# sarphiv/nerf-experiments

Measured on AMD Instinct MI355X. Metric: ray-samples/sec (coarse+fine), training step, higher is better.
Workload: dtype fp32

## Files before the change

include/nerf_amd.h:

```cpp
#ifndef NERF_AMD_H
#define NERF_AMD_H

#include <stdint.h>
#include <stddef.h>

#ifdef __cplusplus
extern "C" {
#endif

#define NERF_OK 0
#define NERF_ERR_INVALID_ARG (-1)
#define NERF_ERR_UNSUPPORTED (-2)
#define NERF_ERR_LAUNCH (-3)
#define NERF_ERR_WORKSPACE (-4)

int nerf_abi_version(void);
const char* nerf_status_string(int status);
int64_t nerf_struct_size(int32_t which);
#define NERF_BUILD_DIAG_FUSED 1
#define NERF_BUILD_DIAG_WGRAD 2
int32_t nerf_build_flags(void);

int nerf_composite_fwd(const float* density, int64_t density_stride,
                       const float* color, int64_t color_stride,
// ... 97 lines not shown
                       float* out, int64_t ldo, int32_t epilogue,
                       const float* aux, int64_t ld_aux, void* stream);
int nerf_linear_wgrad_x3(const float* dY, int64_t ld_dy, int32_t N,
                         const nerf_seg* segs, int32_t n_segs, int64_t M,
                         void* workspace, size_t workspace_bytes, int32_t passes, void* stream);
int nerf_linear_wgrad_x3_rows(const float* dY, int64_t ld_dy, const nerf_seg* segs, int64_t M0,
                              const float* dY1, int64_t ld_dy1, const nerf_seg* segs1, int64_t M1,
                              int32_t n_segs, int32_t N, void* workspace, size_t workspace_bytes,
                              int32_t passes, void* stream);
int nerf_linear_wgrad_x3_rays(const float* dY, int64_t ld_dy, const nerf_seg* segs, int64_t M0,
                              const float* dY1, int64_t ld_dy1, const nerf_seg* segs1, int64_t M1,
                              int32_t n_segs, int32_t N, void* workspace, size_t workspace_bytes,
                              float* raysum, int32_t samples_per_ray0, int32_t samples_per_ray1,
                              int32_t passes, void* stream);
int nerf_linear_wgrad_x3_rows_q(const float* dY, int64_t ld_dy, const nerf_seg* segs, int64_t M0,
                                const float* dY1, int64_t ld_dy1, const nerf_seg* segs1, int64_t M1,
                                int32_t n_segs, int32_t N, void* workspace, size_t workspace_bytes,
                                int32_t passes, uint32_t x_split_mask, void* stream);
int nerf_linear_wgrad_x3_rays_q(const float* dY, int64_t ld_dy, const nerf_seg* segs, int64_t M0,
                                const float* dY1, int64_t ld_dy1, const nerf_seg* segs1, int64_t M1,
                                int32_t n_segs, int32_t N, void* workspace, size_t workspace_bytes,
                                float* raysum, int32_t samples_per_ray0, int32_t samples_per_ray1,
                                int32_t passes, uint32_t x_split_mask, void* stream);
int nerf_pack_weight_x3(const float* W, int32_t N, int32_t K_orig, const int32_t* col_map,
                        int32_t Kp, void* Wp_x, void* Wt_x, int32_t ldwt, void* stream);

#define NERF_FUSED_MAX_LAYERS 16
typedef struct nerf_fused_layer {
    int32_t type;
    int32_t N;
    int32_t nb;
    int32_t relu;
    int32_t nseg;
    int32_t seg_kb[2];
    int32_t seg_k[2];
    int32_t seg_rd[2];
    int32_t seg_rows[2];
    int32_t chunk_units;
    int32_t col_idx;
    int64_t seg_ld[2];
    const float* seg_ptr[2];
    float* out;
    int64_t ldo;
    uint8_t* mask;
    float* col_out;
    int64_t img_off;
// ... 245 lines not shown
```

nerf-experiments_amd/csrc/linear_x3.hip:

```cpp
#include "common.h"
#include "param_act.h"

using namespace nerf;

typedef float f32x16 __attribute__((ext_vector_type(16)));
typedef float f4 __attribute__((ext_vector_type(4)));
typedef __bf16 bf16x8 __attribute__((ext_vector_type(8)));
typedef __bf16 bf16x4 __attribute__((ext_vector_type(4)));
typedef unsigned short u16x8 __attribute__((ext_vector_type(8)));

namespace {

constexpr int BK = 32;
constexpr int LDB = BK;

__device__ __forceinline__ int swz(int row, int slot) {
    return (row >> 1) * 64 + ((((row & 1) << 2) | slot) ^ ((row >> 2) & 7)) * 8;
}
constexpr int MAX_SEGS = 4;

struct SegList {
    const float* ptr[MAX_SEGS];
    int64_t ld[MAX_SEGS];
    int k[MAX_SEGS];
// ... 1444 lines not shown
            const int k = wc * 32 * JN + j * 32 + (lane & 31);
#pragma unroll
            for (int r = 0; r < 16; ++r) {
                const int n = wr * 128 + i * 32 + (r & 3) + 8 * (r >> 2) + 4 * (lane >> 5);
                if (n < npad && k < kpad) slab[(size_t)n * kpad + k] = acc[i][j][r];
            }
        }
    float* red = reinterpret_cast<float*>(smem);
    *reinterpret_cast<f4*>(red + (op * 4 + (wave & 3)) * 256 + 4 * lane) = op == 0 ? dbp : dacc;
    if (ROW257 && op == 1 && lane == 0) red[2048 + (wave & 3)] = dbx;
    __syncthreads();
    if (t < 256) {
        const float s = ((red[t] + red[256 + t]) + red[512 + t]) + red[768 + t];
        if (t < npad) a.db_slab[(size_t)split * npad + t] = s;
    } else if (ROW257) {
        const int c = t - 256;
        const float* x = red + 1024;
        slab[(size_t)256 * kpad + c] = ((x[c] + x[256 + c]) + x[512 + c]) + x[768 + c];
        if (c == 0)
            a.db_slab[(size_t)split * npad + 256] = ((red[2048] + red[2049]) + red[2050]) + red[2051];
    }
#undef WT_SRC_ROW
#undef WT_YD_ROW
}

constexpr int SN_T = 512;
constexpr int SN_U = 8;
template <int N4>
__global__ __launch_bounds__(SN_T) void linear_wgrad_smalln_kernel(TNArgs a, int kpad) {
    extern __shared__ __attribute__((aligned(16))) float sn_part[];
    const int split = blockIdx.x;
    const int mbeg = split * a.m_per_split;
    const int mend = min(mbeg + a.m_per_split, a.M);
    const int ktot = a.X.ktot;
    const int qw = ktot >> 2;
    const int rg = SN_T / qw;
    const int t = threadIdx.x;
    const int g = t / qw, q = t - g * qw;
    const bool live = g < rg;
    int xs = 0, xoff = 0;
#pragma unroll
    for (int i = 0; i < MAX_SEGS; ++i)
        if (i < a.X.n && 4 * q >= a.X.koff[i] && 4 * q < a.X.koff[i] + a.X.kp[i]) { xs = i; xoff = 4 * q - a.X.koff[i]; }
    const bool col_ok = live && xoff < pick4(a.X.k, xs);
    const float* xp0 = pick4(a.X.ptr, xs) + xoff;
    const int64_t xld0 = pick4(a.X.ld, xs);
// ... 496 lines not shown
                                           int32_t n_segs, int32_t N, void* workspace, size_t workspace_bytes,
                                           float* raysum, int32_t samples_per_ray0, int32_t samples_per_ray1,
                                           int32_t passes, uint32_t x_split_mask, void* stream) {
    NERF_REQUIRE(raysum != nullptr);
    return wgrad_x3_rows_impl(dY, ld_dy, segs, M0, dY1, ld_dy1, segs1, M1, n_segs, N, workspace, workspace_bytes,
                              raysum, samples_per_ray0, samples_per_ray1, passes, x_split_mask, stream);
}

extern "C" int nerf_linear_wgrad_x3_rays(const float* dY, int64_t ld_dy, const nerf_seg* segs, int64_t M0,
                                         const float* dY1, int64_t ld_dy1, const nerf_seg* segs1, int64_t M1,
                                         int32_t n_segs, int32_t N, void* workspace, size_t workspace_bytes,
                                         float* raysum, int32_t samples_per_ray0, int32_t samples_per_ray1,
                                         int32_t passes, void* stream) {
    return nerf_linear_wgrad_x3_rays_q(dY, ld_dy, segs, M0, dY1, ld_dy1, segs1, M1, n_segs, N, workspace,
                                       workspace_bytes, raysum, samples_per_ray0, samples_per_ray1, passes, 0u, stream);
}

extern "C" int nerf_linear_wgrad_x3(const float* dY, int64_t ld_dy, int32_t N, const nerf_seg* segs, int32_t n_segs,
                                    int64_t M, void* workspace, size_t workspace_bytes, int32_t passes, void* stream) {
    return nerf_linear_wgrad_x3_rows(dY, ld_dy, segs, M, nullptr, 0, nullptr, 0, n_segs, N, workspace,
                                     workspace_bytes, passes, stream);
}

extern "C" int nerf_pack_weight_x3(const float* W, int32_t N, int32_t K_orig, const int32_t* col_map, int32_t Kp,
                                   void* Wp_x, void* Wt_x, int32_t ldwt, void* stream) {
    NERF_REQUIRE(W && col_map && N >= 1 && K_orig >= 1 && Kp >= 1 && (Kp % BK) == 0);
    const int npad = ((N + 127) / 128) * 128;
    if (Wt_x) NERF_REQUIRE(ldwt >= ((N + 31) / 32) * 32 && (ldwt % BK) == 0);
    const int kpad_rows = ((Kp + 127) / 128) * 128 + 128;
    int64_t total = (int64_t)npad * Kp;
    if (Wt_x) {
        const int64_t pad_total = (int64_t)(kpad_rows - Kp) * ldwt;
        if (pad_total > total) total = pad_total;
    }
    hipLaunchKernelGGL(pack_weight_x3_kernel, dim3((unsigned)((total + 255) / 256)), dim3(256), 0, as_stream(stream), W,
                       N, K_orig, col_map, Kp, npad, reinterpret_cast<__bf16*>(Wp_x), reinterpret_cast<__bf16*>(Wt_x),
                       ldwt, kpad_rows);
    NERF_CHECK_LAUNCH();
    return NERF_OK;
}

extern "C" __attribute__((visibility("hidden"))) int32_t nerf_tu_build_flags_linear_x3(void) {
    return NERF_TU_BUILD_FLAGS;
}
```

nerf-experiments_amd/nerf_amd/_lib.py:

```python
from __future__ import annotations

import ctypes
import os

import torch

_HERE = os.path.dirname(os.path.abspath(__file__))
LIB_PATH = os.environ.get("NERF_AMD_LIB", os.path.join(_HERE, "libnerf_amd.so"))

c_f = ctypes.c_float
c_i32 = ctypes.c_int32
c_i64 = ctypes.c_int64
c_u32 = ctypes.c_uint32
c_u64 = ctypes.c_uint64
c_vp = ctypes.c_void_p
c_sz = ctypes.c_size_t

NERF_EPI_BIAS = 1
NERF_EPI_RELU = 2
NERF_EPI_MASK = 4
NERF_EPI_ACCUM = 8
NERF_EPI_MASKBITS = 16
NERF_EPI_MASKOUT = 32
NERF_EPI_NO_PERSIST = 256
# ... 191 lines not shown
                                c_i32, c_vp, c_i64, c_vp]),
    "nerf_linear_wgrad_workspace": (c_sz, [c_i64, c_i32, c_i32]),
    "nerf_linear_wgrad": (c_i32, [c_vp, c_i64, c_i32, ctypes.POINTER(NerfSeg), c_i32, c_i64, c_vp, c_sz, c_vp]),
    "nerf_linear_wgrad_reduce": (c_i32, [c_i64, c_i32, c_i32, c_i32, c_vp, c_vp, c_vp, c_i64, c_vp, c_i32, c_vp]),
    "nerf_pack_weight": (c_i32, [c_vp, c_i32, c_i32, c_vp, c_i32, c_vp, c_vp, c_i32, c_vp]),
    "nerf_linear_fwd_x3": (c_i32, [ctypes.POINTER(NerfSeg), c_i32, c_i64, c_vp, c_i32, c_i32, c_vp, c_vp,
                                   c_i64, c_i32, c_vp, c_i64, c_vp]),
    "nerf_linear_gauss_workspace": (c_sz, [c_i64, c_i32]),
    "nerf_linear_gauss_x3": (c_i32, [ctypes.POINTER(NerfSeg), c_i32, c_i64, c_vp, c_i32, c_i32, c_vp, c_vp, c_i64,
                                     c_i32, c_vp, c_vp, c_i64, c_vp, c_i64, c_vp, c_i32, c_vp, c_sz, c_vp]),
    "nerf_linear_wgrad_x3": (c_i32, [c_vp, c_i64, c_i32, ctypes.POINTER(NerfSeg), c_i32, c_i64, c_vp, c_sz, c_i32,
                                     c_vp]),
    "nerf_linear_wgrad_x3_rows": (c_i32, [c_vp, c_i64, ctypes.POINTER(NerfSeg), c_i64, c_vp, c_i64,
                                          ctypes.POINTER(NerfSeg), c_i64, c_i32, c_i32, c_vp, c_sz, c_i32, c_vp]),
    "nerf_linear_wgrad_x3_rays": (c_i32, [c_vp, c_i64, ctypes.POINTER(NerfSeg), c_i64, c_vp, c_i64,
                                          ctypes.POINTER(NerfSeg), c_i64, c_i32, c_i32, c_vp, c_sz, c_vp, c_i32,
                                          c_i32, c_i32, c_vp]),
    "nerf_linear_wgrad_x3_rows_q": (c_i32, [c_vp, c_i64, ctypes.POINTER(NerfSeg), c_i64, c_vp, c_i64,
                                            ctypes.POINTER(NerfSeg), c_i64, c_i32, c_i32, c_vp, c_sz, c_i32, c_u32,
                                            c_vp]),
    "nerf_linear_wgrad_x3_rays_q": (c_i32, [c_vp, c_i64, ctypes.POINTER(NerfSeg), c_i64, c_vp, c_i64,
                                            ctypes.POINTER(NerfSeg), c_i64, c_i32, c_i32, c_vp, c_sz, c_vp, c_i32,
                                            c_i32, c_i32, c_u32, c_vp]),
    "nerf_pack_weight_x3": (c_i32, [c_vp, c_i32, c_i32, c_vp, c_i32, c_vp, c_vp, c_i32, c_vp]),
    "nerf_mlp_fused_fwd": (c_i32, [ctypes.POINTER(NerfFusedLayer), c_i32, c_vp, c_i64,
                                   ctypes.POINTER(NerfFusedEncoding), c_vp]),
    "nerf_mlp_fused_render": (c_i32, [ctypes.POINTER(NerfFusedLayer), c_i32, c_vp, c_i64,
                                      ctypes.POINTER(NerfFusedEncoding), ctypes.POINTER(NerfFusedComposite), c_vp]),
    "nerf_mlp_fused_run": (c_i32, [ctypes.POINTER(NerfFusedLayer), c_i32, c_vp, c_i64, ctypes.POINTER(NerfFusedEncoding),
                                   ctypes.POINTER(NerfFusedComposite), c_i32, c_vp]),
    "nerf_struct_size": (c_i64, [c_i32]),
    "nerf_build_flags": (c_i32, []),
    "nerf_fused_pack": (c_i32, [ctypes.POINTER(c_vp), c_i32, c_vp, c_vp, c_i64, c_vp, c_vp]),
    "nerf_hashgrid_fwd": (c_i32, [ctypes.POINTER(NerfHashgridParams), c_vp, c_vp, c_vp, c_vp, c_vp, c_i64, c_i32,
                                  c_vp, c_vp, c_i64, c_vp]),
    "nerf_kabsch": (c_i32, [c_vp, c_vp, c_i32, c_i32, c_vp, c_vp, c_vp, c_vp, c_vp]),
    "nerf_pose_rays_fwd": (c_i32, [c_vp, c_vp, c_i32, c_vp, c_vp, c_vp, c_i64, c_f, c_vp, c_vp, c_vp, c_vp, c_vp]),
    "nerf_pose_rays_bwd": (c_i32, [c_vp, c_i32, c_vp, c_vp, c_i64, c_f, c_vp, c_vp, c_vp, c_vp, c_vp, c_vp, c_vp,
                                   c_vp, c_vp]),
    "nerf_prop_cdf": (c_i32, [c_vp, c_i64, c_i64, c_i32, c_vp, c_i64, c_vp]),
    "nerf_prop_sample": (c_i32, [c_vp, c_i64, c_vp, c_i64, c_i64, c_i32, c_i32, c_i32, c_u64, c_u64, c_i32, c_f,
                                 c_f, c_vp, c_vp, c_i64, c_vp]),
    "nerf_prop_loss": (c_i32, [c_vp, c_vp, c_i64, c_vp, c_vp, c_i64, c_i64, c_i32, c_i32, c_f, c_vp, c_f, c_vp,
                               c_i64, c_vp]),
    "nerf_hashgrid_workspace": (c_sz, [ctypes.POINTER(NerfHashgridParams)]),
    "nerf_hashgrid_workspace_n": (c_sz, [ctypes.POINTER(NerfHashgridParams), c_i64]),
# ... 71 lines not shown
```

nerf-experiments_amd/nerf_amd/kernels.py:

```python
from __future__ import annotations

import ctypes
import os
from typing import Sequence

import torch

from . import _lib
from ._lib import NerfPEParams, NerfSeg


class KernelTimer:

    def __init__(self):
        self.records = []

    def bracket(self, tag: str, flops: float = 0.0, nbytes: float = 0.0, fn: str | None = None, launches: int = 1):
        start = torch.cuda.Event(enable_timing=True)
        end = torch.cuda.Event(enable_timing=True)
        start.record()
        self.records.append((tag, flops, nbytes, start, end, fn or tag, launches))
        return end

    def summary(self, by: str = "tag"):
# ... 563 lines not shown
        raise ValueError("linear_wgrad_x3_rows: the blocks' segments differ in width")
    a0, a1 = make_segs(segs), make_segs(segs1)
    kt = sum(k for _, k, _ in segs)
    kpad = sum(pad32(k) for _, k, _ in segs)
    wide = wgrad_single_tile(N4, kpad)
    end = TIMER.bracket("linear_wgrad_x3", 2.0 * (M + M1) * N4 * kt,
                        4.0 * (M + M1) * N4 + _segs_bytes(segs, M) + _segs_bytes(segs1, M1) + 4.0 * N4 * kt,
                        fn=WGRAD_TILE_FN if wide else
                        ("linear_wgrad_smalln_kernel" if N4 <= 16 else "linear_wgrad_x3_kernel")) \
        if TIMER is not None else None
    if x_split_mask:
        st = _lib.load().nerf_linear_wgrad_x3_rows_q(_ptr(dY), dY.stride(0), a0, M, _ptr(dY1), dY1.stride(0), a1, M1,
                                                     len(segs), N4, _ptr(workspace),
                                                     workspace.numel() * workspace.element_size(), passes,
                                                     x_split_mask, _stream(dY.device))
    else:
        st = _lib.load().nerf_linear_wgrad_x3_rows(_ptr(dY), dY.stride(0), a0, M, _ptr(dY1), dY1.stride(0), a1, M1,
                                                   len(segs), N4, _ptr(workspace),
                                                   workspace.numel() * workspace.element_size(), passes,
                                                   _stream(dY.device))
    if end is not None:
        end.record()
    _lib.check(st, "nerf_linear_wgrad_x3_rows")


def linear_wgrad_x3_rays(blocks, N4: int, workspace: torch.Tensor, raysum: torch.Tensor, S0: int, S1: int,
                        passes: int = 3, x_split_mask: int = 0) -> None:
    (dY, segs, M), (dY1, segs1, M1) = blocks
    a0, a1 = make_segs(segs), make_segs(segs1)
    kt = sum(k for _, k, _ in segs)
    if raysum.shape[1] != N4 or not raysum.is_contiguous():
        raise ValueError("linear_wgrad_x3_rays: raysum must be contiguous [rays, N4]")
    end = TIMER.bracket("linear_wgrad_x3", 2.0 * (M + M1) * N4 * kt,
                        4.0 * (M + M1) * N4 + _segs_bytes(segs, M) + _segs_bytes(segs1, M1) + 4.0 * N4 * kt
                        + 4.0 * raysum.numel(), fn=WGRAD_TILE_FN) \
        if TIMER is not None else None
    if x_split_mask:
        st = _lib.load().nerf_linear_wgrad_x3_rays_q(_ptr(dY), dY.stride(0), a0, M, _ptr(dY1), dY1.stride(0), a1, M1,
                                                     len(segs), N4, _ptr(workspace),
                                                     workspace.numel() * workspace.element_size(), _ptr(raysum), S0,
                                                     S1, passes, x_split_mask, _stream(dY.device))
    else:
        st = _lib.load().nerf_linear_wgrad_x3_rays(_ptr(dY), dY.stride(0), a0, M, _ptr(dY1), dY1.stride(0), a1, M1,
                                                   len(segs), N4, _ptr(workspace),
                                                   workspace.numel() * workspace.element_size(), _ptr(raysum), S0,
                                                   S1, passes, _stream(dY.device))
# ... 751 lines not shown
```

nerf-experiments_amd/nerf_amd/mlp.py:

```python
from __future__ import annotations

import math
import os
from dataclasses import dataclass, field

import torch
import torch.nn as nn

from . import kernels as K
from . import mlp_fused
from ._lib import (NERF_EPI_ACCUM, NERF_EPI_BIAS, NERF_EPI_MASK, NERF_EPI_MASKBITS, NERF_EPI_MASKOUT,
                   NERF_EPI_RELU, NERF_EPI_TANH, NERF_EPI_TANH_BWD)


def matmul_precision() -> str:
    if PRECISION_OVERRIDE is not None:
        return PRECISION_OVERRIDE
    p = torch.get_float32_matmul_precision()
    return "fp32" if p == "highest" else ("x1" if p == "medium" else "x3")


def is_split(prec: str) -> bool:
    return prec in ("x3", "x1")

# ... 110 lines not shown
        return None
    rows = [(0, nrow)] if nrow <= 257 else [(n0, min(256, nrow - n0)) for n0 in range(0, nrow, 256)]
    groups, cur, used = [], [], 0
    for j, (_, k, rd) in enumerate(segs):
        if kp[j] > 256 and rd != 1:
            return None
        for c0 in range(0, k, 256):
            c1 = min(c0 + 256, k)
            w = K.pad32(c1 - c0)
            if used + w > 256:
                groups.append(cur)
                cur, used = [], 0
            cur.append((j, c0, c1))
            used += w
    groups.append(cur)
    gk = [sum(K.pad32(c1 - c0) for _, c0, c1 in g) for g in groups]
    if len(rows) > 1 and min(gk) <= 128:
        return None
    if any(not (nb > 128 or k > 128) for _, nb in rows for k in gk):
        return None
    return rows, groups


def _wgrad_tiles(blocks, nrow: int, N4: int, lp, workspace, gW, gb, acc, split, npass: int, q=()) -> None:
    rows, groups = split
    Mt = sum(M for _, _, M in blocks)
    poff = [0]
    for _, k, _ in blocks[0][1]:
        poff.append(poff[-1] + K.pad32(k))

    def piece(segs, j, c0, c1):
        t, k, rd = segs[j]
        return (t, k, rd) if (c0, c1) == (0, k) else (t[:, c0:c1], c1 - c0, rd)

    whole = len(rows) == 1
    for n0, nb in rows:
        nr = nrow if whole else nb
        n4 = N4 if whole else nb
        nvalid = lp.N if whole else min(nb, lp.N - n0)
        for gi, g in enumerate(groups):
            pb = [(dZ if whole else dZ[:, n0:n0 + nb], [piece(segs, j, c0, c1) for j, c0, c1 in g], M)
                  for dZ, segs, M in blocks]
            p0 = poff[g[0][0]] + g[0][1]
            kp = sum(K.pad32(c1 - c0) for _, c0, c1 in g)
            ws = _wgrad_workspace(workspace, Mt, n4, kp)
            qm = _qmask(q, [j for j, _, _ in g])
            if len(pb) > 1:
                K.linear_wgrad_x3_rows(pb, nr, ws, passes=npass, x_split_mask=qm)
            else:
                K.linear_wgrad_x3(pb[0][0], nr, pb[0][1], pb[0][2], ws, passes=npass, x_split_mask=qm)
            K.linear_wgrad_reduce(Mt, n4, kp, nvalid, ws, lp.col_map[p0:p0 + kp], gW[n0:n0 + nvalid],
                                  gb[n0:n0 + nvalid] if gi == 0 else None, accumulate=acc)


def _qmask(q, js) -> int:
    return sum(1 << i for i, j in enumerate(js) if j < len(q) and q[j])


def _wgrad_x3(blocks, nrow: int, N4: int, lp, workspace, gW, gb, acc, npass: int, q=()) -> None:
    segs = blocks[0][1]
    rsplit = _ray_split(blocks, N4) if nrow == N4 else None
    tsplit = _tile_split(segs, nrow) if rsplit is None else None
    if rsplit is not None:
        _wgrad_rays(blocks, N4, lp, workspace, gW, gb, acc, rsplit, npass, q)
    elif tsplit is not None:
        _wgrad_tiles(blocks, nrow, N4, lp, workspace, gW, gb, acc, tsplit, npass, q)
    else:
        Mt = sum(M for _, _, M in blocks)
        qm = _qmask(q, range(len(segs)))
        ws = _wgrad_workspace(workspace, Mt, N4, lp.Kp)
        if len(blocks) > 1:
            K.linear_wgrad_x3_rows(blocks, nrow, ws, passes=npass, x_split_mask=qm)
        else:
            K.linear_wgrad_x3(blocks[0][0], nrow, segs, blocks[0][2], ws, passes=npass, x_split_mask=qm)
        K.linear_wgrad_reduce(Mt, N4, lp.Kp, lp.N, ws, lp.col_map, gW, gb, accumulate=acc)


def wgrad_launches(segs, nrow: int, N4: int, M: int, rays: bool = True):
    rsplit = _ray_split([(None, segs, M)], N4) if rays and nrow == N4 else None
    if rsplit is not None:
        n = len(segs) - 1
        return [(N4, [(j, K.pad32(segs[j][1])) for j in range(n)]), (N4, [(n, K.pad32(segs[n][1]))])]
    tsplit = _tile_split(segs, nrow)
    if tsplit is not None:
        rows, groups = tsplit
        return [(nrow if len(rows) == 1 else nb, [(j, K.pad32(c1 - c0)) for j, c0, c1 in g])
                for _, nb in rows for g in groups]
    return [(nrow, [(j, K.pad32(k)) for j, (_, k, _) in enumerate(segs)])]


SAVE_SPLIT = False


def split_layers(plan, M: int, dir_rd: int) -> frozenset:
    if not SAVE_SPLIT or CAPTURE is not None or not mlp_fused.dgrad_eligible(plan, M):
        return frozenset()
    cols = {li for li, _ in plan.column_outputs}
    out = set()
    for l, lp in enumerate(plan.layers[:-1]):
        if lp.N > 256 or l in plan.outputs or l in cols or lp.keeps_pre or lp.tanh:
            continue
        readers = [(c, si) for c, cl in enumerate(plan.layers) for si, s in enumerate(cl.sources)
                   if s.kind == "act" and s.layer == l]
        if not readers or any(cl.residual == l for cl in plan.layers):
            continue
        ok = True
        for c, si in readers:
            cl = plan.layers[c]
            if c != l + 1 or si != 0 or cl.N == 257:
                ok = False
                break
# ... 416 lines not shown
                    if comp_chain and l == sl and plan.layers[l].out_ld == 260:
                        continue
                    dY[l][:, 256:].zero_()
            if comp_chain:
                comp_rt = (comp, g_rgb, dY[L - 1], dY[sl][:, 256:] if sl >= 0 else None, sl)
            x_out = {}
            for (l, _, _, _, x, *_rest) in fd.steps:
                if x is not None:
                    x_out[l] = torch.empty(M, x.k_pad, device=dev, dtype=torch.float32)
            fd.run(M, g_head, dY, ctx.masks, g_cols, x_out, comp=comp_rt, passes=passes(ctx.prec))
            for (l, _, _, _, x, *_rest) in fd.steps:
                if x is None:
                    continue
                if x.kind == "pos":
                    dpos = x_out[l] if dpos is None else dpos.add_(x_out[l])
                else:
                    ddir = x_out[l] if ddir is None else ddir.add_(x_out[l])

        ws_bytes = 0
        for lp in plan.layers:
            ws_bytes = max(ws_bytes, K.linear_wgrad_workspace_bytes(M, (lp.N + 3) // 4 * 4, lp.Kp))
        workspace = torch.empty((ws_bytes + 3) // 4, device=dev, dtype=torch.float32)

        for li in range(L - 1, -1, -1):
            lp = plan.layers[li]
            if col_grads[li]:
                if dY[li] is None:
                    dY[li] = torch.zeros(M, lp.out_ld, device=dev, dtype=torch.float32)
                elif not owned[li]:
                    dY[li] = dY[li].clone()
                for c, g in col_grads[li]:
                    dY[li][:, c] += g
            dZ = dY[li]
            w = lp.module.weight
            sink = ctx.sink
            if dZ is None:
                if sink is not None:
                    for t in (w, lp.module.bias):
                        g, acc = sink.target(t)
                        if not acc:
                            g.zero_()
                        sink.landed(t)
                    layer_grads[li] = [None, None]
                else:
                    layer_grads[li] = [torch.zeros_like(w), torch.zeros_like(lp.module.bias)]
                layer_grads[li] += [torch.zeros_like(p) for p in lp.pact]
                continue
# ... 16 lines not shown
                segs.append((t, s.k_seg, rd))
            N4 = (lp.N + 3) // 4 * 4
            nrow = lp.N if (lp.N == 257 and WGRAD_ROW257) else N4
            q = tuple(s.kind == "act" and s.layer in ctx.split for s in lp.sources)
            merge = sink is not None and is_split(ctx.prec) and MERGE_PASSES and not gs
            prev = sink.stash.pop((id(plan), li), (None, None))[0] if merge else None
            if merge and prev is None and sink.remaining(w) >= 2:
                sink.stash[(id(plan), li)] = ((dZ, segs, M, nrow, N4, lp, passes(ctx.prec), q), _flush_wgrad)
                layer_grads[li] = [None, None]
            else:
                if sink is not None:
                    gW, acc = sink.target(w)
                    gb, acc_b = sink.target(lp.module.bias)
                    if acc != acc_b:
                        raise RuntimeError("direct gradient sink: weight and bias of one layer out of step")
                else:
                    gW, gb, acc = torch.empty_like(w), torch.empty_like(lp.module.bias), False
                npass = passes(ctx.prec)
                if prev is not None and prev[7] != q:
                    _wgrad_x3([(prev[0], prev[1], prev[2])], nrow, N4, lp, workspace, gW, gb, acc, npass, prev[7])
                    _wgrad_x3([(dZ, segs, M)], nrow, N4, lp, workspace, gW, gb, True, npass, q)
                elif is_split(ctx.prec):
                    wblocks = [(prev[0], prev[1], prev[2]), (dZ, segs, M)] if prev is not None else [(dZ, segs, M)]
                    _wgrad_x3(wblocks, nrow, N4, lp, workspace, gW, gb, acc, npass, q)
                else:
                    K.linear_wgrad(dZ, N4, segs, M, workspace)
                    K.linear_wgrad_reduce(M, N4, lp.Kp, lp.N, workspace, lp.col_map, gW, gb, accumulate=acc)
                if sink is not None:
                    for _ in range(2 if prev is not None else 1):
                        sink.landed(w)
                        sink.landed(lp.module.bias)
                    gW = gb = None
                layer_grads[li] = [gW, gb] + (gs if gs is not None else [])
            if chain:
                continue
            lp.pack(ctx.prec, forward=False)
            a_seg = [(dZ, lp.out_ld, 1)]
            for s, koff in zip(lp.sources, lp.koffs):
                if s.kind == "act":
                    j = s.layer
                    prod = plan.layers[j]
                    if (GAUSS_EPILOGUE and prod.keeps_pre and plan.contributors[j] == 1 and dY[j] is None
                            and not prod.relu and is_split(ctx.prec) and prod.bwd_epilogue_fits(s.k_valid)):
                        dz = torch.empty(M, prod.out_ld, device=dev, dtype=torch.float32)
                        gsj = [torch.empty_like(p) for p in prod.pact]
                        if prod.linear_act_x3(a_seg, M, lp.Wtx, lp.ldwt, s.k_valid, dz, z=pre[j], grads=gsj,
                                              w_row_offset=koff):
                            dY[j] = dz
                            gauss_done[j] = gsj
                            continue
                    epi = 0
                    aux = None
                    if prod.tanh:
                        epi |= NERF_EPI_TANH_BWD
# ... 10 lines not shown
                            aux = acts[j]
                    fresh = dY[j] is None
                    if fresh:
                        dY[j] = torch.empty(M, prod.out_ld, device=dev, dtype=torch.float32)
                    else:
                        epi |= NERF_EPI_ACCUM
                    lp.gemm(ctx.prec, a_seg, M, True, s.k_valid, None, dY[j], epi, aux=aux, row_offset=koff)
                    if fresh and prod.out_ld > s.k_valid:
                        dY[j][:, s.k_valid:].zero_()
                elif s.kind == "pos" and need_pos:
                    if dpos is None:
                        dpos = torch.empty(M, s.k_pad, device=dev, dtype=torch.float32)
                        epi = 0
                    else:
                        epi = NERF_EPI_ACCUM
                    lp.gemm(ctx.prec, a_seg, M, True, s.k_pad, None, dpos, epi, row_offset=koff)
                elif s.kind == "dir" and need_dir:
                    if ddir is None:
                        ddir = torch.empty(M, s.k_pad, device=dev, dtype=torch.float32)
                        epi = 0
                    else:
                        epi = NERF_EPI_ACCUM
                    lp.gemm(ctx.prec, a_seg, M, True, s.k_pad, None, ddir, epi, row_offset=koff)
        if ddir is not None and ctx.dir_rd > 1:
            ddir = ddir.view(-1, ctx.dir_rd, ddir.shape[1]).sum(dim=1)
        if dpos is not None and dpos.shape[1] != ctx.n_pos_cols:
            dpos = dpos[:, :ctx.n_pos_cols]
        if ddir is not None and ddir.shape[1] != ctx.n_dir_cols:
            ddir = ddir[:, :ctx.n_dir_cols]
        param_grads = [g for lg in layer_grads for g in lg]
        return (None, None, dpos, ddir, None, *param_grads)


def nerf_model_plan(n_segments: int, model_segments: nn.ModuleList, model_color: nn.Sequential,
                    hidden_dim: int, pos_dim: int, dir_dim: int, delayed_direction: bool,
                    delayed_density: bool) -> tuple[MLPPlan, int, int]:
    layers: list[LayerPlan] = []
    pos_src = Source("pos", pos_dim, K.pad32(pos_dim))
    dir_src = Source("dir", dir_dim, K.pad32(dir_dim))
    prev = -1
    for i in range(n_segments):
        seg = model_segments[i]
        linears = [m for m in seg.modules() if isinstance(m, nn.Linear)] if isinstance(seg, nn.Sequential) \
            else [seg]
        for j, lin in enumerate(linears):
            srcs: list[Source] = []
# ... 24 lines not shown
```

Measured before the change: 72.15 million.

## Pair two weight-gradient GEMMs sharing the same position input into one kernel

Adds a paired wgrad kernel that reads the shared X (position encoding) tile once and computes weight gradients for two layers (late skip-connection piece and early layer) in a single launch, each using half the waves. The Python backward defers (holds) the late layer's pos-segment wgrad until the matching early layer is reached, then launches the pair. This is meant to remove one pass over X and one launch, and to improve occupancy for the small-K GEMMs. In exchange it allocates an extra workspace per call, makes the bookkeeping more complex, and changes when gradients are marked landed.

After: 72.76 million (median of 6 runs). No clear change (+0.8%).

```diff
diff --git a/include/nerf_amd.h b/include/nerf_amd.h
--- a/include/nerf_amd.h
+++ b/include/nerf_amd.h
@@ -143,6 +143,12 @@
                                 int32_t n_segs, int32_t N, void* workspace, size_t workspace_bytes,
                                 float* raysum, int32_t samples_per_ray0, int32_t samples_per_ray1,
                                 int32_t passes, uint32_t x_split_mask, void* stream);
+int nerf_linear_wgrad_x3_pair(const float* dYa, int64_t ld_dya, const float* dYa1, int64_t ld_dya1,
+                              int32_t Na, int32_t bias_a, void* workspace_a, size_t workspace_a_bytes,
+                              const float* dYb, int64_t ld_dyb, const float* dYb1, int64_t ld_dyb1,
+                              int32_t Nb, int32_t bias_b, void* workspace_b, size_t workspace_b_bytes,
+                              const nerf_seg* segs, int64_t M0, const nerf_seg* segs1, int64_t M1,
+                              int32_t n_segs, int32_t passes, uint32_t x_split_mask, void* stream);
 int nerf_pack_weight_x3(const float* W, int32_t N, int32_t K_orig, const int32_t* col_map,
                         int32_t Kp, void* Wp_x, void* Wt_x, int32_t ldwt, void* stream);
 
diff --git a/nerf-experiments_amd/csrc/linear_x3.hip b/nerf-experiments_amd/csrc/linear_x3.hip
--- a/nerf-experiments_amd/csrc/linear_x3.hip
+++ b/nerf-experiments_amd/csrc/linear_x3.hip
@@ -1490,6 +1490,244 @@
     }
 #undef WT_SRC_ROW
 #undef WT_YD_ROW
+}
+
+constexpr int PT_IMG = 6 * WT_T * 512;
+constexpr int PT_RELAY = 2 * 4 * 4 * 64 * 16;
+struct TNPairArgs {
+    const float* dY[2][2]; int64_t lddy[2][2]; int N[2];
+    const float* X[2]; int64_t ldx[2]; int k, kp;
+    int M, M0, m_per_split;
+    float* slab[2]; float* db_slab[2];
+    int npad[2], kpad;
+};
+
+template <bool X1>
+__global__ __launch_bounds__(512, 1) __attribute__((amdgpu_waves_per_eu(2, 2))) void linear_wgrad_x3_pair_kernel(
+    TNPairArgs a) {
+    __shared__ __attribute__((aligned(16))) char smem[2 * PT_IMG + PT_RELAY];
+    typedef const __attribute__((address_space(1))) f4* gf4p;
+    const int split = blockIdx.x;
+    const int mbeg = split * a.m_per_split;
+    const int mend = min(mbeg + a.m_per_split, a.M);
+    const int M0 = a.M0;
+    const int steps = mbeg < mend ? (mend - mbeg + WT_T - 1) / WT_T : 0;
+    const int t = threadIdx.x;
+    const int wave = __builtin_amdgcn_readfirstlane(t >> 6), lane = t & 63;
+    const int dop = wave >> 2;
+    const int lr = 4 * (wave & 3);
+
+    const int N = dop ? a.N[1] : a.N[0];
+    unsigned cmask = 0;
+#pragma unroll
+    for (int e = 0; e < 4; ++e) cmask |= (4 * lane + e < N ? 1u : 0u) << e;
+    const unsigned voff = 4u * (unsigned)(4 * lane < N ? 4 * lane : 0);
+    const wt_gcp ub0 = (wt_gcp)(dop ? a.dY[1][0] : a.dY[0][0]), ub1 = (wt_gcp)(dop ? a.dY[1][1] : a.dY[0][1]);
+    const int64_t uld0 = 4 * (dop ? a.lddy[1][0] : a.lddy[0][0]), uld1 = 4 * (dop ? a.lddy[1][1] : a.lddy[0][1]);
+    const int lpr = a.kp >> 2;
+    const bool x_on = lane < 2 * lpr;
+    const int xsel = x_on && lane >= lpr ? 1 : 0;
+    const int xcq = x_on ? lane - xsel * lpr : 0;
+    const int xrow = 4 * (wave >> 1) + (wave & 1) + 2 * xsel;
+    const bool xcol_ok = 4 * xcq < a.k;
+    const unsigned xvoff = xcol_ok ? 16u * (unsigned)xcq : 0u;
+    const wt_gcp xb0 = (wt_gcp)a.X[0], xb1 = (wt_gcp)a.X[1];
+    const int64_t xld0 = 4 * a.ldx[0], xld1 = 4 * a.ldx[1];
+    auto x_src = [=](int i) __attribute__((always_inline)) {
+        int m = mbeg + i * WT_T + xrow;
+        m = m < mend ? m : mbeg;
+        const bool b1f = m >= M0;
+        const unsigned r = (unsigned)(b1f ? m - M0 : m);
+        return (b1f ? xb1 : xb0) + (int64_t)r * (b1f ? xld1 : xld0) + xvoff;
+    };
+#define PT_SRC_ROW_U(i, q) wt_src_row_u(ub0, ub1, uld0, uld1, M0, mbeg, mend, (i) * WT_T + lr + (q), voff)
+    f4 ra[4], rb[4], xa, xb;
+    auto issue = [&](int i, f4 (&r)[4], f4& x) __attribute__((always_inline)) {
+#pragma unroll
+        for (int q = 0; q < 4; ++q) r[q] = __builtin_nontemporal_load((gf4p)PT_SRC_ROW_U(i, q));
+        x = __builtin_nontemporal_load((gf4p)x_src(i));
+    };
+
+    f4 dbp = {0.f, 0.f, 0.f, 0.f};
+    f4 dbq = {0.f, 0.f, 0.f, 0.f};
+    const bool narrow = N <= 128;
+    char* const relay = smem + 2 * PT_IMG + ((wave >> 1) * 4 * 64 + lane) * 16;
+    unsigned woff[4];
+#pragma unroll
+    for (int q = 0; q < 4; ++q) woff[q] = wt_off(dop, 0, lr + q, 4 * lane);
+    const unsigned xwoff = wt_off(2, 0, xrow, 4 * xcq);
+    const bool cols_full = __ballot(cmask != 0xfu) == 0;
+
+    typedef __bf16 bf16x2 __attribute__((ext_vector_type(2)));
+    typedef float f2 __attribute__((ext_vector_type(2)));
+    typedef unsigned u2 __attribute__((ext_vector_type(2)));
+    auto put = [](char* p, u32x4 w) __attribute__((always_inline)) {
+        const f4 v = __builtin_bit_cast(f4, w);
+        u2 h, l;
+#pragma unroll
+        for (int pp = 0; pp < 2; ++pp) {
+            const f2 x2 = {v[2 * pp], v[2 * pp + 1]};
+            const unsigned hp = __builtin_bit_cast(unsigned, __builtin_convertvector(x2, bf16x2));
+            const f2 hv = {__builtin_bit_cast(float, hp << 16), __builtin_bit_cast(float, hp & 0xffff0000u)};
+            h[pp] = hp;
+            l[pp] = __builtin_bit_cast(unsigned, __builtin_convertvector(x2 - hv, bf16x2));
+        }
+        *reinterpret_cast<u2*>(p) = h;
+        *reinterpret_cast<u2*>(p + WT_T * 512) = l;
+    };
+    auto convert = [&](auto parc, auto prevc, int i, const f4 (&r)[4], const f4& x) __attribute__((always_inline)) {
+        constexpr int PAR = decltype(parc)::value;
+        constexpr bool PREV = decltype(prevc)::value != 0;
+        const int valid = mend - (mbeg + i * WT_T);
+        char* const img = smem + (i & 1) * PT_IMG;
+        u32x4 rw[4];
+#pragma unroll
+        for (int q = 0; q < 4; ++q) rw[q] = __builtin_bit_cast(u32x4, r[q]);
+        if (!(cols_full && valid >= WT_T)) {
+#pragma unroll
+            for (int q = 0; q < 4; ++q) {
+                const unsigned rm = lr + q < valid ? cmask : 0u;
+#pragma unroll
+                for (int e = 0; e < 4; ++e) rw[q][e] &= (unsigned)__builtin_amdgcn_sbfe((int)rm, (unsigned)e, 1u);
+            }
+        }
+        if (!narrow) {
+#pragma unroll
+            for (int q = 0; q < 4; ++q) dbp += __builtin_bit_cast(f4, rw[q]);
+        } else if (wave & 1) {
+#pragma unroll
+            for (int q = 0; q < 4; ++q)
+                *reinterpret_cast<f4*>(relay + PAR * (PT_RELAY / 2) + q * 64 * 16) = __builtin_bit_cast(f4, rw[q]);
+        } else {
+            if constexpr (PREV) {
+                f4& prev = PAR ? dbp : dbq;
+#pragma unroll
+                for (int q = 0; q < 4; ++q)
+                    prev += *reinterpret_cast<const f4*>(relay + (1 - PAR) * (PT_RELAY / 2) + q * 64 * 16);
+            }
+            f4& cur = PAR ? dbq : dbp;
+#pragma unroll
+            for (int q = 0; q < 4; ++q) cur += __builtin_bit_cast(f4, rw[q]);
+        }
+#pragma unroll
+        for (int q = 0; q < 4; ++q) put(img + woff[q], rw[q]);
+        const unsigned xm = xcol_ok && xrow < valid ? ~0u : 0u;
+        u32x4 xw = __builtin_bit_cast(u32x4, x);
+#pragma unroll
+        for (int e = 0; e < 4; ++e) xw[e] &= xm;
+        if (x_on) put(img + xwoff, xw);
+    };
+
+    const int wr = wave >> 2, wc = wave & 3;
+    const bool act_k = wc * 32 < a.kp;
+    const bool active0 = act_k && wr * 128 < a.N[0], active1 = act_k && wr * 128 < a.N[1];
+    const int G = lane >> 4, qq = (lane & 15) >> 2, pq = lane & 3;
+    unsigned ya_off[4];
+#pragma unroll
+    for (int ii = 0; ii < 4; ++ii) ya_off[ii] = wt_off(0, 0, 8 * (G >> 1) + qq, wr * 128 + 32 * ii + 16 * (G & 1) + 4 * pq);
+    const unsigned xa_off = wt_off(2, 0, 8 * (G >> 1) + qq, wc * 32 + 16 * (G & 1) + 4 * pq);
+    auto frag = [&](const char* img, unsigned off) __attribute__((always_inline)) {
+        const s16x4 lo4 = __builtin_amdgcn_ds_read_tr16_b64_v4i16((lds_s16x4_t*)(img + off));
+        const s16x4 hi4 = __builtin_amdgcn_ds_read_tr16_b64_v4i16((lds_s16x4_t*)(img + off + 4 * 512));
+        return __builtin_bit_cast(bf16x8, __builtin_shufflevector(lo4, hi4, 0, 1, 2, 3, 4, 5, 6, 7));
+    };
+    f32x16 acc[2][4];
+#pragma unroll
+    for (int o = 0; o < 2; ++o)
+#pragma unroll
+        for (int i = 0; i < 4; ++i)
+#pragma unroll
+            for (int r = 0; r < 16; ++r) acc[o][i][r] = 0.f;
+    auto mfma_step = [&](int i) __attribute__((always_inline)) {
+        const char* img = smem + (i & 1) * PT_IMG;
+        const bf16x8 xh = frag(img, xa_off), xl = frag(img, xa_off + WT_T * 512);
+#pragma unroll
+        for (int o = 0; o < 2; ++o) {
+            if (o == 0 ? active0 : active1) {
+                const char* yimg = img + o * (2 * WT_T * 512);
+                bf16x8 yh[4], yl[4];
+#pragma unroll
+                for (int ii = 0; ii < 4; ++ii) {
+                    yh[ii] = frag(yimg, ya_off[ii]);
+                    yl[ii] = frag(yimg, ya_off[ii] + WT_T * 512);
+                }
+#pragma unroll
+                for (int ii = 0; ii < 4; ++ii) acc[o][ii] = mfma_w<X1>(yh[ii], yl[ii], xh, xl, acc[o][ii]);
+            }
+        }
+    };
+    auto barrier = []() __attribute__((always_inline)) {
+        asm volatile("s_waitcnt lgkmcnt(0)" ::: "memory");
+        __builtin_amdgcn_s_barrier();
+        __builtin_amdgcn_sched_barrier(0);
+    };
+    auto run = [&](auto earlyc) __attribute__((always_inline)) {
+        constexpr bool EARLY = decltype(earlyc)::value != 0;
+        issue(0, ra, xa);
+        issue(1, rb, xb);
+        convert(wt_tag<0>{}, wt_tag<0>{}, 0, ra, xa);
+        issue(2, ra, xa);
+        barrier();
+        int i = 0;
+        for (; i + 1 < steps; i += 2) {
+            if (EARLY && act_k) mfma_step(i);
+            convert(wt_tag<1>{}, wt_tag<1>{}, i + 1, rb, xb);
+            issue(i + 3, rb, xb);
+            if (!EARLY && act_k) mfma_step(i);
+            barrier();
+            if (EARLY && act_k) mfma_step(i + 1);
+            convert(wt_tag<0>{}, wt_tag<1>{}, i + 2, ra, xa);
+            issue(i + 4, ra, xa);
+            if (!EARLY && act_k) mfma_step(i + 1);
+            barrier();
+        }
+        if (i < steps) {
+            if (act_k) mfma_step(i);
+            barrier();
+        }
+    };
+    if (steps > 0) {
+        if (dop)
+            run(wt_tag<1>{});
+        else
+            run(wt_tag<0>{});
+        if (narrow && !(wave & 1)) {
+#pragma unroll
+            for (int q = 0; q < 4; ++q) dbp += *reinterpret_cast<const f4*>(relay + q * 64 * 16);
+        }
+    }
+
+#pragma unroll
+    for (int o = 0; o < 2; ++o) {
+        const int npad = a.npad[o], kpad = a.kpad;
+        float* slab = a.slab[o] + (size_t)split * npad * kpad;
+        const int k = wc * 32 + (lane & 31);
+#pragma unroll
+        for (int i = 0; i < 4; ++i)
+#pragma unroll
+            for (int r = 0; r < 16; ++r) {
+                const int n = wr * 128 + i * 32 + (r & 3) + 8 * (r >> 2) + 4 * (lane >> 5);
+                if (n < npad && k < kpad) slab[(size_t)n * kpad + k] = acc[o][i][r];
+            }
+    }
+    float* red = reinterpret_cast<float*>(smem);
+    if (!narrow) {
+        *reinterpret_cast<f4*>(red + wave * 256 + 4 * lane) = dbp;
+    } else if (!(wave & 1)) {
+        const int g = (wave & 3) >> 1;
+        *reinterpret_cast<f4*>(red + (dop * 4 + g) * 256 + 4 * lane) = dbp;
+        *reinterpret_cast<f4*>(red + (dop * 4 + 2 + g) * 256 + 4 * lane) = dbq;
+    }
+    __syncthreads();
+    {
+        const int o = t >> 8, c = t & 255;
+        const float* p = red + o * 1024;
+        const float s = ((p[c] + p[256 + c]) + p[512 + c]) + p[768 + c];
+        float* db = o ? a.db_slab[1] : a.db_slab[0];
+        const int npad = o ? a.npad[1] : a.npad[0];
+        if (db != nullptr && c < npad) db[(size_t)split * npad + c] = s;
+    }
+#undef PT_SRC_ROW_U
 }
 
 constexpr int SN_T = 512;
@@ -2032,6 +2270,78 @@
                                      workspace_bytes, passes, stream);
 }
 
+extern "C" int nerf_linear_wgrad_x3_pair(const float* dYa, int64_t ld_dya, const float* dYa1, int64_t ld_dya1,
+                                         int32_t Na, int32_t bias_a, void* workspace_a, size_t workspace_a_bytes,
+                                         const float* dYb, int64_t ld_dyb, const float* dYb1, int64_t ld_dyb1,
+                                         int32_t Nb, int32_t bias_b, void* workspace_b, size_t workspace_b_bytes,
+                                         const nerf_seg* segs, int64_t M0, const nerf_seg* segs1, int64_t M1,
+                                         int32_t n_segs, int32_t passes, uint32_t x_split_mask, void* stream) {
+    NERF_REQUIRE(passes == 1 || passes == 3);
+    const int64_t M = M0 + M1;
+    NERF_REQUIRE(M0 >= 0 && M1 >= 0 && M >= 1 && M < (1ll << 31));
+    NERF_REQUIRE(n_segs == 1 && x_split_mask == 0u);
+    NERF_REQUIRE(Na >= 1 && Na <= 256 && Nb >= 1 && Nb <= 256);
+    NERF_REQUIRE(!(SMALLN_ON && (Na <= 16 || Nb <= 16)));
+    SegList L;
+    NERF_REQUIRE(build_segs(segs, n_segs, L));
+    NERF_REQUIRE(L.ktot <= 128 && L.row_div[0] == 1);
+    NERF_REQUIRE(dYa && aligned16(dYa) && (ld_dya % 4) == 0 && ld_dya >= (Na + 3) / 4 * 4);
+    NERF_REQUIRE(dYb && aligned16(dYb) && (ld_dyb % 4) == 0 && ld_dyb >= (Nb + 3) / 4 * 4);
+    TNPairArgs a{};
+    a.dY[0][0] = a.dY[0][1] = dYa;
+    a.lddy[0][0] = a.lddy[0][1] = ld_dya;
+    a.dY[1][0] = a.dY[1][1] = dYb;
+    a.lddy[1][0] = a.lddy[1][1] = ld_dyb;
+    a.X[0] = a.X[1] = L.ptr[0];
+    a.ldx[0] = a.ldx[1] = L.ld[0];
+    a.N[0] = Na;
+    a.N[1] = Nb;
+    a.k = L.k[0];
+    a.kp = L.kp[0];
+    a.M = (int)M;
+    a.M0 = (int)M;
+    if (M1 > 0) {
+        SegList L1;
+        NERF_REQUIRE(build_segs(segs1, n_segs, L1) && L1.k[0] == L.k[0] && L1.row_div[0] == 1);
+        NERF_REQUIRE(dYa1 && aligned16(dYa1) && (ld_dya1 % 4) == 0 && ld_dya1 >= (Na + 3) / 4 * 4);
+        NERF_REQUIRE(dYb1 && aligned16(dYb1) && (ld_dyb1 % 4) == 0 && ld_dyb1 >= (Nb + 3) / 4 * 4);
+        a.dY[0][1] = dYa1;
+        a.lddy[0][1] = ld_dya1;
+        a.dY[1][1] = dYb1;
+        a.lddy[1][1] = ld_dyb1;
+        a.X[1] = L1.ptr[0];
+        a.ldx[1] = L1.ld[0];
+        a.M0 = (int)M0;
+    }
+    const int ntk = (L.ktot + TB - 1) / TB;
+    int splits = 0;
+    void* const wsp[2] = {workspace_a, workspace_b};
+    const size_t wsb[2] = {workspace_a_bytes, workspace_b_bytes};
+    const int want_bias[2] = {bias_a, bias_b};
+    for (int o = 0; o < 2; ++o) {
+        const int N = a.N[o], ntn = (N + TB - 1) / TB;
+        const int s = nerf_wgrad_choose_splits(M, nerf_wgrad_split_tiles(N, L.ktot));
+        NERF_REQUIRE(o == 0 || s == splits);
+        splits = s;
+        if (!wsp[o] || wsb[o] < nerf_linear_wgrad_workspace(M, N, L.ktot) || !aligned16(wsp[o])) return NERF_ERR_WORKSPACE;
+        a.slab[o] = reinterpret_cast<float*>(wsp[o]);
+        a.db_slab[o] = want_bias[o] ? a.slab[o] + (size_t)splits * ntn * TB * (size_t)ntk * TB : nullptr;
+        a.npad[o] = ntn * TB;
+    }
+    NERF_REQUIRE(workspace_a != workspace_b);
+    a.kpad = ntk * TB;
+    int64_t mps = (M + splits - 1) / splits;
+    mps = ((mps + TBM - 1) / TBM) * TBM;
+    a.m_per_split = (int)mps;
+    const dim3 grid((unsigned)splits), block(512);
+    if (passes == 1)
+        hipLaunchKernelGGL(linear_wgrad_x3_pair_kernel<true>, grid, block, 0, as_stream(stream), a);
+    else
+        hipLaunchKernelGGL(linear_wgrad_x3_pair_kernel<false>, grid, block, 0, as_stream(stream), a);
+    NERF_CHECK_LAUNCH();
+    return NERF_OK;
+}
+
 extern "C" int nerf_pack_weight_x3(const float* W, int32_t N, int32_t K_orig, const int32_t* col_map, int32_t Kp,
                                    void* Wp_x, void* Wt_x, int32_t ldwt, void* stream) {
     NERF_REQUIRE(W && col_map && N >= 1 && K_orig >= 1 && Kp >= 1 && (Kp % BK) == 0);
diff --git a/nerf-experiments_amd/nerf_amd/_lib.py b/nerf-experiments_amd/nerf_amd/_lib.py
--- a/nerf-experiments_amd/nerf_amd/_lib.py
+++ b/nerf-experiments_amd/nerf_amd/_lib.py
@@ -237,6 +237,10 @@
     "nerf_linear_wgrad_x3_rays_q": (c_i32, [c_vp, c_i64, ctypes.POINTER(NerfSeg), c_i64, c_vp, c_i64,
                                             ctypes.POINTER(NerfSeg), c_i64, c_i32, c_i32, c_vp, c_sz, c_vp, c_i32,
                                             c_i32, c_i32, c_u32, c_vp]),
+    "nerf_linear_wgrad_x3_pair": (c_i32, [c_vp, c_i64, c_vp, c_i64, c_i32, c_i32, c_vp, c_sz,
+                                          c_vp, c_i64, c_vp, c_i64, c_i32, c_i32, c_vp, c_sz,
+                                          ctypes.POINTER(NerfSeg), c_i64, ctypes.POINTER(NerfSeg), c_i64, c_i32,
+                                          c_i32, c_u32, c_vp]),
     "nerf_pack_weight_x3": (c_i32, [c_vp, c_i32, c_i32, c_vp, c_i32, c_vp, c_vp, c_i32, c_vp]),
     "nerf_mlp_fused_fwd": (c_i32, [ctypes.POINTER(NerfFusedLayer), c_i32, c_vp, c_i64,
                                    ctypes.POINTER(NerfFusedEncoding), c_vp]),
diff --git a/nerf-experiments_amd/nerf_amd/kernels.py b/nerf-experiments_amd/nerf_amd/kernels.py
--- a/nerf-experiments_amd/nerf_amd/kernels.py
+++ b/nerf-experiments_amd/nerf_amd/kernels.py
@@ -609,6 +609,34 @@
     if end is not None:
         end.record()
     _lib.check(st, "nerf_linear_wgrad_x3_rows")
+
+
+def linear_wgrad_x3_pair(blocks_a, Na: int, ws_a: torch.Tensor, bias_a: bool, blocks_b, Nb: int, ws_b: torch.Tensor,
+                         bias_b: bool, passes: int = 3, x_split_mask: int = 0) -> None:
+    if len(blocks_a) != len(blocks_b) or any(a[2] != b[2] for a, b in zip(blocks_a, blocks_b)):
+        raise ValueError("linear_wgrad_x3_pair: the two operands' row blocks differ")
+    (dYa, segs, M) = blocks_a[0]
+    dYb = blocks_b[0][0]
+    two = len(blocks_a) > 1
+    dYa1, segs1, M1 = blocks_a[1] if two else (None, None, 0)
+    dYb1 = blocks_b[1][0] if two else None
+    a0 = make_segs(segs)
+    a1 = make_segs(segs1) if two else None
+    kt = sum(k for _, k, _ in segs)
+    Mt = M + M1
+    end = TIMER.bracket("linear_wgrad_x3", 2.0 * Mt * (Na + Nb) * kt,
+                        4.0 * Mt * (Na + Nb) + _segs_bytes(segs, M) + (_segs_bytes(segs1, M1) if two else 0.0)
+                        + 4.0 * (Na + Nb) * kt, fn="linear_wgrad_x3_pair_kernel") \
+        if TIMER is not None else None
+    st = _lib.load().nerf_linear_wgrad_x3_pair(
+        _ptr(dYa), dYa.stride(0), _ptr(dYa1), dYa1.stride(0) if two else 0, Na, int(bool(bias_a)), _ptr(ws_a),
+        ws_a.numel() * ws_a.element_size(),
+        _ptr(dYb), dYb.stride(0), _ptr(dYb1), dYb1.stride(0) if two else 0, Nb, int(bool(bias_b)), _ptr(ws_b),
+        ws_b.numel() * ws_b.element_size(),
+        a0, M, a1, M1, len(segs), passes, x_split_mask, _stream(dYa.device))
+    if end is not None:
+        end.record()
+    _lib.check(st, "nerf_linear_wgrad_x3_pair")
 
 
 def linear_wgrad_x3_rays(blocks, N4: int, workspace: torch.Tensor, raysum: torch.Tensor, S0: int, S1: int,
diff --git a/nerf-experiments_amd/nerf_amd/mlp.py b/nerf-experiments_amd/nerf_amd/mlp.py
--- a/nerf-experiments_amd/nerf_amd/mlp.py
+++ b/nerf-experiments_amd/nerf_amd/mlp.py
@@ -156,7 +156,7 @@
     return rows, groups
 
 
-def _wgrad_tiles(blocks, nrow: int, N4: int, lp, workspace, gW, gb, acc, split, npass: int, q=()) -> None:
+def _wgrad_tiles(blocks, nrow: int, N4: int, lp, workspace, gW, gb, acc, split, npass: int, q=(), hold=None):
     rows, groups = split
     Mt = sum(M for _, _, M in blocks)
     poff = [0]
@@ -177,8 +177,13 @@
                   for dZ, segs, M in blocks]
             p0 = poff[g[0][0]] + g[0][1]
             kp = sum(K.pad32(c1 - c0) for _, c0, c1 in g)
+            qm = _qmask(q, [j for j, _, _ in g])
+            if whole and hold is not None and gi == hold["gi"] and qm == 0 and nr == n4:
+                hold["held"] = dict(blocks=pb, nr=nr, n4=n4, kp=kp, nvalid=nvalid, cols=lp.col_map[p0:p0 + kp],
+                                    gW=gW[n0:n0 + nvalid], gb=gb[n0:n0 + nvalid] if gi == 0 else None, acc=acc,
+                                    npass=npass)
+                continue
             ws = _wgrad_workspace(workspace, Mt, n4, kp)
-            qm = _qmask(q, [j for j, _, _ in g])
             if len(pb) > 1:
                 K.linear_wgrad_x3_rows(pb, nr, ws, passes=npass, x_split_mask=qm)
             else:
@@ -187,18 +192,59 @@
                                   gb[n0:n0 + nvalid] if gi == 0 else None, accumulate=acc)
 
 
+def _run_held(h, workspace) -> None:
+    Mt = sum(M for _, _, M in h["blocks"])
+    ws = _wgrad_workspace(workspace, Mt, h["n4"], h["kp"])
+    pb = h["blocks"]
+    if len(pb) > 1:
+        K.linear_wgrad_x3_rows(pb, h["nr"], ws, passes=h["npass"])
+    else:
+        K.linear_wgrad_x3(pb[0][0], h["nr"], pb[0][1], pb[0][2], ws, passes=h["npass"])
+    K.linear_wgrad_reduce(Mt, h["n4"], h["kp"], h["nvalid"], ws, h["cols"], h["gW"], h["gb"], accumulate=h["acc"])
+
+
+def _pairs_with(h, blocks, nrow: int, N4: int, npass: int, q) -> bool:
+    if h is None or nrow != N4 or not 128 < N4 <= 256 or any(q) or npass != h["npass"]:
+        return False
+    hb = h["blocks"]
+    if len(hb) != len(blocks):
+        return False
+    for (_, hs, hM), (_, s, M) in zip(hb, blocks):
+        if len(s) != 1 or len(hs) != 1 or hM != M or s[0][1:] != hs[0][1:] or s[0][2] != 1:
+            return False
+        if s[0][0].data_ptr() != hs[0][0].data_ptr() or s[0][0].stride() != hs[0][0].stride():
+            return False
+    return True
+
+
+def _wgrad_pair(blocks, N4: int, lp, workspace, gW, gb, acc, npass: int, h) -> None:
+    Mt = sum(M for _, _, M in blocks)
+    ws_a = _wgrad_workspace(workspace, Mt, N4, lp.Kp)
+    need_b = K.linear_wgrad_workspace_bytes(Mt, h["n4"], h["kp"])
+    ws_b = torch.empty((need_b + 3) // 4, device=ws_a.device, dtype=torch.float32)
+    K.linear_wgrad_x3_pair(blocks, N4, ws_a, True, h["blocks"], h["nr"], ws_b, h["gb"] is not None, passes=npass)
+    K.linear_wgrad_reduce(Mt, N4, lp.Kp, lp.N, ws_a, lp.col_map, gW, gb, accumulate=acc)
+    K.linear_wgrad_reduce(Mt, h["n4"], h["kp"], h["nvalid"], ws_b, h["cols"], h["gW"], h["gb"], accumulate=h["acc"])
+
+
 def _qmask(q, js) -> int:
     return sum(1 << i for i, j in enumerate(js) if j < len(q) and q[j])
 
 
-def _wgrad_x3(blocks, nrow: int, N4: int, lp, workspace, gW, gb, acc, npass: int, q=()) -> None:
+def _wgrad_x3(blocks, nrow: int, N4: int, lp, workspace, gW, gb, acc, npass: int, q=(), hold=None, held=None):
     segs = blocks[0][1]
     rsplit = _ray_split(blocks, N4) if nrow == N4 else None
     tsplit = _tile_split(segs, nrow) if rsplit is None else None
     if rsplit is not None:
         _wgrad_rays(blocks, N4, lp, workspace, gW, gb, acc, rsplit, npass, q)
     elif tsplit is not None:
-        _wgrad_tiles(blocks, nrow, N4, lp, workspace, gW, gb, acc, tsplit, npass, q)
+        if hold is None:
+            _wgrad_tiles(blocks, nrow, N4, lp, workspace, gW, gb, acc, tsplit, npass, q)
+        else:
+            _wgrad_tiles(blocks, nrow, N4, lp, workspace, gW, gb, acc, tsplit, npass, q, hold=hold)
+    elif _pairs_with(held, blocks, nrow, N4, npass, q):
+        _wgrad_pair(blocks, N4, lp, workspace, gW, gb, acc, npass, held)
+        return True
     else:
         Mt = sum(M for _, _, M in blocks)
         qm = _qmask(q, range(len(segs)))
@@ -221,6 +267,62 @@
         return [(nrow if len(rows) == 1 else nb, [(j, K.pad32(c1 - c0)) for j, c0, c1 in g])
                 for _, nb in rows for g in groups]
     return [(nrow, [(j, K.pad32(k)) for j, (_, k, _) in enumerate(segs)])]
+
+
+WGRAD_PAIR = True
+
+
+def wgrad_layer_desc(plan, dir_rd: int):
+    out = []
+    for lp in plan.layers:
+        segs = [(s.kind if s.kind != "act" else ("act", s.layer), s.k_seg, dir_rd if s.kind == "dir" else 1)
+                for s in lp.sources]
+        N4 = (lp.N + 3) // 4 * 4
+        out.append((segs, lp.N if (lp.N == 257 and WGRAD_ROW257) else N4, N4))
+    return out
+
+
+def wgrad_pairs(layers, M: int, rays: bool = True) -> dict:
+    pairs, taken = {}, set()
+    if not WGRAD_PAIR:
+        return pairs
+    for late in range(len(layers) - 1, 0, -1):
+        segs, nrow, N4 = layers[late]
+        if (rays and nrow == N4 and _ray_split([(None, segs, M)], N4) is not None) or _tile_split(segs, nrow) is None:
+            continue
+        for gi, (nr, piece) in enumerate(wgrad_launches(segs, nrow, N4, M, rays)):
+            if nr != N4 or nr > 256 or len(piece) != 1:
+                continue
+            j, kp = piece[0]
+            key, k, rd = segs[j]
+            if key != "pos" or rd != 1 or kp != K.pad32(k) or kp > 128 or not K.wgrad_single_tile(nr, kp):
+                continue
+            early = next((e for e in range(late) if e not in taken and layers[e][0] == [(key, k, rd)]
+                          and layers[e][1] == layers[e][2] and 128 < layers[e][2] <= 256), None)
+            if early is not None:
+                pairs[late] = (gi, early)
+                taken.update((early, late))
+                break
+    return pairs
+
+
+def wgrad_plan_launches(layers, M: int, rays: bool = True):
+    pairs = wgrad_pairs(layers, M, rays)
+    by_early = {e: (late, gi) for late, (gi, e) in pairs.items()}
+    out = []
+    for li in range(len(layers) - 1, -1, -1):
+        segs, nrow, N4 = layers[li]
+        launches = wgrad_launches(segs, nrow, N4, M, rays)
+        if li in by_early:
+            late, gi = by_early[li]
+            ls, lnrow, lN4 = layers[late]
+            out.append(("pair", li, late, wgrad_launches(ls, lnrow, lN4, M, rays)[gi][1]))
+            continue
+        for gi, (nr, piece) in enumerate(launches):
+            if li in pairs and pairs[li][0] == gi:
+                continue
+            out.append(("single", li, nr, piece))
+    return out
 
 
 SAVE_SPLIT = False
@@ -683,7 +785,25 @@
             ws_bytes = max(ws_bytes, K.linear_wgrad_workspace_bytes(M, (lp.N + 3) // 4 * 4, lp.Kp))
         workspace = torch.empty((ws_bytes + 3) // 4, device=dev, dtype=torch.float32)
 
+        pairs = wgrad_pairs(wgrad_layer_desc(plan, ctx.dir_rd), M) if is_split(ctx.prec) else {}
+        held = None
+
+        def resolve_held(ran: bool) -> None:
+            nonlocal held
+            if held is None:
+                return
+            h, _, params, n = held
+            held = None
+            if not ran:
+                _run_held(h, workspace)
+            if ctx.sink is not None:
+                for _ in range(n):
+                    for t in params:
+                        ctx.sink.landed(t)
+
         for li in range(L - 1, -1, -1):
+            if held is not None and held[1] > li:
+                resolve_held(False)
             lp = plan.layers[li]
             if col_grads[li]:
                 if dY[li] is None:
@@ -746,14 +866,22 @@
                     _wgrad_x3([(dZ, segs, M)], nrow, N4, lp, workspace, gW, gb, True, npass, q)
                 elif is_split(ctx.prec):
                     wblocks = [(prev[0], prev[1], prev[2]), (dZ, segs, M)] if prev is not None else [(dZ, segs, M)]
-                    _wgrad_x3(wblocks, nrow, N4, lp, workspace, gW, gb, acc, npass, q)
+                    if held is not None and held[1] == li:
+                        resolve_held(_wgrad_x3(wblocks, nrow, N4, lp, workspace, gW, gb, acc, npass, q,
+                                               held=held[0]) is True)
+                    else:
+                        hold = {"gi": pairs[li][0]} if li in pairs else None
+                        _wgrad_x3(wblocks, nrow, N4, lp, workspace, gW, gb, acc, npass, q, hold=hold)
+                        if hold is not None and "held" in hold:
+                            held = (hold["held"], pairs[li][1], (w, lp.module.bias), 2 if prev is not None else 1)
                 else:
                     K.linear_wgrad(dZ, N4, segs, M, workspace)
                     K.linear_wgrad_reduce(M, N4, lp.Kp, lp.N, workspace, lp.col_map, gW, gb, accumulate=acc)
                 if sink is not None:
-                    for _ in range(2 if prev is not None else 1):
-                        sink.landed(w)
-                        sink.landed(lp.module.bias)
+                    if not (held is not None and held[2][0] is w):
+                        for _ in range(2 if prev is not None else 1):
+                            sink.landed(w)
+                            sink.landed(lp.module.bias)
                     gW = gb = None
                 layer_grads[li] = [gW, gb] + (gs if gs is not None else [])
             if chain:
@@ -810,6 +938,7 @@
                     else:
                         epi = NERF_EPI_ACCUM
                     lp.gemm(ctx.prec, a_seg, M, True, s.k_pad, None, ddir, epi, row_offset=koff)
+        resolve_held(False)
         if ddir is not None and ctx.dir_rd > 1:
             ddir = ddir.view(-1, ctx.dir_rd, ddir.shape[1]).sum(dim=1)
         if dpos is not None and dpos.shape[1] != ctx.n_pos_cols:
```
